# RS2002/PianoBart

Measured on AMD Instinct MI355X. Metric: Octuple tokens/sec/GPU (seq=1024, 12L/768d) pretrain step; %MFMA peak, higher is better.
Workload: dtype bf16

## Files before the change

pianobart_amd/csrc/pb_api_internal.h:

```cpp
#pragma once
#include <hip/hip_runtime.h>
#include "../../include/pianobart_hip.h"

int pb_gemm2_try(const pb_gemm_desc* d, void* stream);
int pb_finalize_rows(const float* partials, int nblk, int d, float* out, void* stream, int nacc = 1, float* out1 = nullptr);
float* pb_defer_alloc(size_t nfloats);
int pb_gemm_x3(const pb_gemm_desc* d, void* stream);
int pb_flash64_fwd(const pb_attn_desc& d, hipStream_t stream);
int pb_flash64_bwd(const pb_attn_desc& d, hipStream_t stream);
int pb_flash1_bwd(const pb_attn_desc& d, hipStream_t stream);
int pb_flash_x3_fwd(const pb_attn_desc& d, hipStream_t stream);
int pb_flash_x3_bwd(const pb_attn_desc& d, hipStream_t stream);
const void* pb_zero_page();
```

pianobart_amd/csrc/pb_gemm.hip:

```cpp
#include "pb_common.h"
#include "pb_api_internal.h"
#include <algorithm>

namespace {

constexpr int BM = 128, BN = 128, NTHREADS = 256;
constexpr int ROW_BYTES = 128;
constexpr int TILE_BYTES = BM * ROW_BYTES;

template <typename T> struct Elem;
template <> struct Elem<bf16_t> { static constexpr int EPV = 8, BK = 64; };
template <> struct Elem<float>  { static constexpr int EPV = 4, BK = 32; };

struct Vec16 { uint32_t w[4]; };

__device__ __forceinline__ int swz(int row) { return ((row >> 1) & 7) ^ ((row >> 4) & 7); }

template <typename T>
__device__ __forceinline__ Vec16 load_vec(const T* __restrict__ base, long off, int nvalid, bool aligned) {
    constexpr int EPV = Elem<T>::EPV;
    Vec16 v = {{0u, 0u, 0u, 0u}};
    if (nvalid <= 0) return v;
    if (aligned && nvalid == EPV) {
        const uint4 q = *reinterpret_cast<const uint4*>(base + off);
// ... 240 lines not shown
    else hipLaunchKernelGGL((gemm_kernel<T, false, false>), grid, block, lds, stream, a);
    PB_LAUNCH_CHECK();
    return 0;
}

}

static int colsum_of_c(const pb_gemm_desc* d, void* stream_) {
    const bool c32 = (d->flags & PB_GEMM_C_F32) || d->dtype == PB_F32;
    return pb_colsum(d->C, d->ldc, d->colsum_out, d->colsum_ws, d->M, d->N, c32 ? PB_F32 : PB_BF16, c32 ? 1 : 0, stream_);
}

extern "C" int pb_gemm(const pb_gemm_desc* d, void* stream_) {
    hipStream_t stream = (hipStream_t)stream_;
    PB_REQUIRE(d != nullptr, "pb_gemm: null descriptor");
    PB_REQUIRE(d->dtype == PB_F32 || d->dtype == PB_BF16 || d->dtype == PB_F32X3, "pb_gemm: bad dtype %d", d->dtype);
    PB_REQUIRE(d->M >= 0 && d->N >= 0 && d->K >= 0, "pb_gemm: negative size");
    if (d->M == 0 || d->N == 0) return 0;
    PB_REQUIRE(d->A && d->B && d->C, "pb_gemm: null operand");
    PB_REQUIRE(!(d->flags & PB_GEMM_GELU) || d->aux_out, "pb_gemm: GELU epilogue needs aux_out");
    PB_REQUIRE(!(d->flags & PB_GEMM_MUL_GELU_GRAD) || d->aux_in, "pb_gemm: gelu-grad epilogue needs aux_in");
    const int nbt = (d->nb1 > 0 ? d->nb1 : 1) * (d->nb2 > 0 ? d->nb2 : 1);
    PB_REQUIRE(!d->colsum_out || (d->colsum_ws && nbt == 1 && d->ldc == d->N && d->N % 4 == 0), "pb_gemm: colsum_out needs colsum_ws, one batch and a dense C with N a multiple of 4");
    if (d->dtype == PB_F32X3) return pb_gemm_x3(d, stream_);
    if (!(d->flags & PB_GEMM_FORCE_V1)) {
        const int r2 = pb_gemm2_try(d, stream_);
        if (r2 < 0) return r2;
        if (r2 == 0) return 0;
        if (r2 == 2) return colsum_of_c(d, stream_);
    }
    if (d->flags & PB_GEMM_ROWDOT) {
        pb_set_error("pb_gemm: PB_GEMM_ROWDOT is only served by the bf16 NT 256x256 kernel (not with PB_GEMM_FORCE_V1, f32, K %% 64 != 0 or operands off 16 bytes)");
        return -2;
    }
    const int esz = d->dtype == PB_BF16 ? 2 : 4, epv = 16 / esz;
    GemmArgs a;
    a.A = d->A; a.B = d->B; a.C = d->C; a.bias = d->bias; a.aux_in = d->aux_in; a.aux_out = d->aux_out;
    a.M = d->M; a.N = d->N; a.K = d->K; a.lda = d->lda; a.ldb = d->ldb; a.ldc = d->ldc; a.ldaux = d->ldaux;
    const int nb1 = d->nb1 > 0 ? d->nb1 : 1;
    a.nb2 = d->nb2 > 0 ? d->nb2 : 1;
    a.sA1 = d->sA1; a.sA2 = d->sA2; a.sB1 = d->sB1; a.sB2 = d->sB2; a.sC1 = d->sC1; a.sC2 = d->sC2;
    a.alpha = d->alpha; a.flags = d->flags;
    auto aligned = [&](const void* p, long ld, long s1, long s2) {
        return ((uintptr_t)p % 16 == 0) && (ld % epv == 0) && (s1 % epv == 0) && (s2 % epv == 0);
    };
    a.a_aligned = aligned(d->A, d->lda, d->sA1, d->sA2);
    a.b_aligned = aligned(d->B, d->ldb, d->sB1, d->sB2);
    a.tiles_m = (d->M + BM - 1) / BM; a.tiles_n = (d->N + BN - 1) / BN;
    PB_REQUIRE((long)nb1 * a.nb2 <= 65535, "pb_gemm: too many batches");
    const int rc = d->dtype == PB_BF16 ? launch_gemm<bf16_t>(a, d->a_kcontig, d->b_kcontig, nb1 * a.nb2, stream)
                                       : launch_gemm<float>(a, d->a_kcontig, d->b_kcontig, nb1 * a.nb2, stream);
    if (rc) return rc;
    return d->colsum_out ? colsum_of_c(d, stream_) : 0;
}

extern "C" int64_t pb_gemm_colsum_ws_floats(int32_t M, int32_t N) {
    const int64_t fused = 2LL * ((M + 255) / 256) * N;
    return std::max<int64_t>(fused, pb_colsum_partials_floats(N));
}
```

pianobart_amd/embedding.py:

```python
from collections import OrderedDict

import numpy as np
import torch

from . import ops, pieces
from ._lib import PBError

STAGES = ('encode', 'pool', 'moments', 'distances', 'knn', 'counts')
D2_BLOCK_BYTES = 64 << 20


def _run(timer, stage, fn, *args, **kw):
    return fn(*args, **kw) if timer is None else timer.run(stage, fn, *args, **kw)


class EmbeddingMixin:
    def embed(self, enc16, emask, timer=None):
        if enc16.device.type != 'cuda':
            raise PBError('pianobart_amd needs HIP device tensors (got %s); there is no CPU path' % enc16.device)
        B, S = int(enc16.shape[0]), int(enc16.shape[1])
        if emask is not None and tuple(emask.shape) != (B, S):
            raise PBError('embed: encoder_attention_mask of shape %s for ids of (%d, %d, 8)' % (tuple(emask.shape), B, S))
        self.bind(enc16.device)
        self._await_updates(2)
        with torch.no_grad():
            enc16 = self.note_ids(enc16.contiguous(), owned=False)
            em = emask.to(torch.float32).contiguous() if emask is not None else None
            _, enc_h = _run(timer, 'encode', self.forward_hidden, enc16, None, em, None, False, 0)
            emb, count = _run(timer, 'pool', ops.pool_rows, enc_h.view(B, S, self.d), em)
        self.check_ids(collective=False)
        return emb, count


def _backbone(model):
    pb = getattr(model, 'pianobart', model)
    if not hasattr(pb, 'embed') or not hasattr(pb, 'layout'):
        raise PBError('embedding: the model must be a PianoBart or a model that holds one as .pianobart (got %s)' % type(model).__name__)
    return pb


def arrange(ids, layout, pad_word, start=None):
    a = pieces.host_ids(ids, layout)
    live = pieces.live_rows(a, layout, start)[1]
    order = np.argsort(~live, axis=1, kind='stable')
    moved = np.take_along_axis(a, order[:, :, None], 1)
    n_live = live.sum(1)
    moved[np.arange(a.shape[1])[None, :] >= n_live[:, None]] = np.asarray(pad_word, dtype=np.int64)
    keep = n_live > 0
    return moved[keep], n_live[keep].astype(np.int64), int((~keep).sum())


def _embed_rows(pb, rows, batch_size, timer=None):
    if isinstance(batch_size, bool) or not isinstance(batch_size, (int, np.integer)) or batch_size < 1:
        raise PBError('embedding: batch_size = %r must be an integer >= 1' % (batch_size,))
    S = rows.shape[1]
    if S > pb.bartConfig.max_position_embeddings:
        raise PBError('embedding: pieces of %d rows exceed max_position_embeddings %d' % (S, pb.bartConfig.max_position_embeddings))
# ... 142 lines not shown
```

pianobart_amd/engine.py:

```python
import os

import numpy as np
import torch

from . import ops, rowpack

from ._lib import LIB, PB_BF16, PB_F32, PB_F32X3, PBError
from .generation import LN_EPS, GenerationMixin, check_prefix, check_samples, sample_seed
from .embedding import EmbeddingMixin
from .scoring import ScoringMixin

_WGRAD_STREAM = int(os.environ.get('PB_WGRAD_STREAM', '7'))
_WG_DXD_256 = int(os.environ.get('PB_WG_DXD_256', '1'))
_WG_TARGET = 192 if _WGRAD_STREAM & 1 else 256
_ROWDOT = int(os.environ.get('PB_ROWDOT', '1'))
_X3_ONEHOT = int(os.environ.get('PB_X3_ONEHOT', '1'))
_DP_RESERVE_CUS = int(os.environ.get('PB_DP_RESERVE_CUS', '0'))
_SIDE_PRIORITY = int(os.environ.get('PB_SIDE_PRIORITY', '0'))
_X3_FLASH = int(os.environ.get('PB_X3_FLASH', '1'))

_RING = 2
_EVENT_MODE = 1
_FWD_GEMM_FLAGS = int(os.environ.get('PB_FWD_GEMM_FLAGS', '32768'))
_PACK_ROWS = int(os.environ.get('PB_PACK_ROWS', '1'))
# ... 210 lines not shown
                    R, C = s.shape
                    rows.append([s.off, R, C, tiles])
                    tiles += -(-R // 64) * -(-C // 64)
                    self.wT[name] = self.PbfT[s.off:s.off + s.numel].view(C, R)
            if rows:
                self._wT_table = torch.tensor(rows, dtype=torch.int32, device=device)
                self._wT_tiles = tiles
        self.Gcur = self.G32
        self.opt_m = self.opt_v = None
        self._versions = None
        self._ws_cache = {}
        self.ptab = torch.zeros(self.lay.tab_total, self.d, dtype=torch.float32, device=device)
        self.dptab = torch.zeros(self.lay.tab_total, self.d, dtype=torch.float32, device=device)
        npart = max(int(LIB.query('pb_ln_partials_floats', self.d)), int(LIB.query('pb_colsum_partials_floats', max(3 * self.d, self.fe, self.fd, self.lay.vocab))),
                    int(LIB.query('pb_ce_partials_floats')), int(LIB.query('pb_norm_partials_floats')))
        self.partials = torch.empty(npart, dtype=torch.float32, device=device)
        self.scal = torch.zeros(64, dtype=torch.float32, device=device)
        w = [len(self.pb.e2w[k]) for k in self.pb.e2w]
        self.loss_w = torch.tensor(w, dtype=torch.float32, device=device)
        self.sos16 = torch.tensor(self.pb.sos_word_np, dtype=torch.int16, device=device)

    def _alias_cross_kv(self, dct):
        if self.ND:
            d2 = 2 * self.d
            for l in range(self.ND):
                dct['dec.%d.wkv_c' % l] = dct['dec.wkv_all'][l * d2:(l + 1) * d2]
                dct['dec.%d.bkv_c' % l] = dct['dec.bkv_all'][l * d2:(l + 1) * d2]

    def refresh_shadow(self, force=False):
        if self.code != PB_BF16:
            return
        ver = sum(p._version for p in self.params)
        if force or ver != self._versions:
            self._await_updates(2)
            ops.cast_f32_to_bf16(self.P32, self.Pbf)
            self._versions = ver
            self._shadow_gen += 1

    def _refresh_wT(self, on_side=False):
        if self._wT_table is None:
            return
        gen = self._shadow_gen
        if on_side and self._side and _WGRAD_STREAM:
            self._event().wait_on(self._side)
            with torch.cuda.stream(self._side):
                ops.transpose_batch_bf16(self.Pbf, self.PbfT, self._wT_table, self._wT_tiles)
                self._wT_done = self._event()
        else:
            ops.transpose_batch_bf16(self.Pbf, self.PbfT, self._wT_table, self._wT_tiles)
            self._wT_done = None
        self._wT_gen = gen

    def _ensure_wT(self):
        if self._wT_table is None:
            return
        if self._wT_gen != self._shadow_gen:
            self._refresh_wT()
        if self._wT_done is not None:
            self._wT_done.wait_on(torch.cuda.current_stream())
            self._wT_done = None

    def _ws(self, B, S):
        key = (B, S)
        ws = self._ws_cache.get(key)
        if ws is not None:
            return ws
        dev, X, d, H = self.device, self.xdt, self.d, self.H
# ... 135 lines not shown
    def forward_hidden(self, enc16, dec16, emask, dmask, train, seed, reuse_encoder=False, dec_embeds=None, pack=None):
        B, S = (pack.B, pack.S) if pack is not None else enc16.shape[:2]
        if S > self.Smax:
            raise PBError('sequence length %d exceeds max_position_embeddings %d' % (S, self.Smax))
        self._fwd_token += 1
        d = self.d
        Te, Td = (pack.Te, pack.Td) if pack is not None else (B * S, B * S)
        ws = self._ws_rows(self._ws(B, S), Te, Td)
        self._cur_ws = ws
        r_enc, r_dec, r_cross = (pack.enc, pack.dec, pack.cross) if pack is not None else (None, None, None)
        ids_e, ids_d = (pack.src_e, pack.src_d) if pack is not None else (None, None)
        p = self.p_drop if train else 0.0
        self._await_updates(0)
        if not self._tables_ready:
            self.refresh_shadow()
            self.build_ptab()
        self._tables_ready = False
        self._kmax = {}
        if self.use_flash and (self.x3 or self.hd in (64, 96, 128)) and pack is None:
            for msk in (emask, dmask):
                if msk is not None and id(msk) not in self._kmax:
                    km = torch.empty(msk.shape[0], dtype=torch.int32, device=msk.device)
                    ops.key_extent(msk, km)
                    self._kmax[id(msk)] = km
        self._kmax_keep = (emask, dmask)
        wf = self.wf
        x = ws['x_enc']
        if not reuse_encoder:
            ops.embed_ln_fwd(enc16, self.ptab, wf['lin.b'], wf['enc.pos'], wf['enc.lne.w'], wf['enc.lne.b'], x, ws['me'], ws['re'], S,
                             LN_EPS, seed, self._site('enc_emb'), p, padded=True, layout=self.lay, row_ids=ids_e)
        T = Te
        for l in range(self.NE if not reuse_encoder else 0):
            L, pf = ws['enc'][l], 'enc.%d.' % l
            if l == 2:
                self._await_updates(1)
            self._linear(x, pf + 'wqkv', pf + 'bqkv', L['qkv'], T, 3 * d, d)
            self._attn_fwd((L['qkv'], 0, 3 * d), (L['qkv'], d, 3 * d), (L['qkv'], 2 * d, 3 * d), (L['ctx'], 0, d), emask, False, B, S, S, L['attn'],
                           rows=r_enc)
            self._linear(L['ctx'], pf + 'wo', pf + 'bo', L['a1'], T, d, d)
            ops.add_ln_fwd(x, L['a1'], wf[pf + 'ln1.w'], wf[pf + 'ln1.b'], L['y1'], L['m1'], L['r1'], LN_EPS, seed, self._site('enc', l, 0), p, row_ids=ids_e)
            self._linear(L['y1'], pf + 'w1', pf + 'b1', L['g'], T, self.fe, d, gelu_aux_out=L['u'])
            self._linear(L['g'], pf + 'w2', pf + 'b2', L['a2'], T, d, self.fe)
            ops.add_ln_fwd(L['y1'], L['a2'], wf[pf + 'ln2.w'], wf[pf + 'ln2.b'], L['y2'], L['m2'], L['r2'], LN_EPS, seed, self._site('enc', l, 1), p, row_ids=ids_e)
            x = L['y2']
        enc_out = x if not reuse_encoder else (ws['enc'][-1]['y2'] if self.NE else x)
        if dec16 is None and dec_embeds is None:
            return None, enc_out
        self._await_updates(2)
        y = ws['x_dec']
        T = Td
        if dec_embeds is None:
            ops.embed_ln_fwd(dec16, self.ptab, wf['lin.b'], wf['dec.pos'], wf['dec.lne.w'], wf['dec.lne.b'], y, ws['md'], ws['rd'], S,
                             LN_EPS, seed, self._site('dec_emb'), p, padded=True, layout=self.lay, row_ids=ids_d)
        else:
            ws['alt_pos'] = wf['dec.pos'][2:2 + S].to(self.xdt).unsqueeze(0).expand(B, S, d).reshape(T, d).contiguous()
            ws['alt_e'] = dec_embeds
            pre = y if p == 0.0 else ws.setdefault('x_dec_pre', torch.empty_like(y))
            ops.add_ln_fwd(ws['alt_pos'], dec_embeds, wf['dec.lne.w'], wf['dec.lne.b'], pre, ws['md'], ws['rd'], LN_EPS, 0, 0, 0.0)
            if p > 0.0:
                ops.dropout(pre, y, seed, self._site('dec_emb'), p)
        kvld = self.ND * 2 * d
        kv_cut = min(_KV_CUT, self.ND)

        def kv_project(l0, l1):
            ops.gemm(enc_out, self.w['dec.wkv_all'], ws['kvc_all'], M=Te, N=(l1 - l0) * 2 * d, K=d, dtype=self.gcode, bias=self.wf['dec.bkv_all'][l0 * 2 * d:],
                     ldc=kvld, b_off=l0 * 2 * d * d, c_off=l0 * 2 * d, dbg=_FWD_GEMM_FLAGS)
        kv_ready = None
        if (_WGRAD_STREAM & 2) and self._side_stream() is not None and self.ND:
            self._event().wait_on(self._side)
            with torch.cuda.stream(self._side):
                kv_project(0, kv_cut)
                kv_ready = [self._event()] * kv_cut
                if self.ND > kv_cut:
                    kv_project(kv_cut, self.ND)
                    kv_ready += [self._event()] * (self.ND - kv_cut)
        elif self.ND:
            kv_project(0, self.ND)
        kv_of = lambda l: ((ws['kvc_all'], l * 2 * d, kvld), (ws['kvc_all'], l * 2 * d + d, kvld))
        sub = pack.sub if pack is not None else None
        sub_layer = None
        for l in range(self.ND):
# ... 321 lines not shown
            gA = self._ffn_ln_bwd(L, pf, self.fe, cur, L['y1'], seed, self._site('enc', l, 1), p, Te, row_ids=ids_e)
            dqkv_e = self._ring('dqkv')[:Te]
            g2 = gy if cur is not gy else galt
            bq = g[pf + 'bqkv']
            fused = self._attn_block_bwd(L, pf, (pf + 'wo', pf + 'bo'), gA, x_in, (L['qkv'], 0, 3 * d), (L['qkv'], d, 3 * d), (L['qkv'], 2 * d, 3 * d),
                                         (dqkv_e, 0, 3 * d), (dqkv_e, d, 3 * d), (dqkv_e, 2 * d, 3 * d), L['ctx'], L['a1'], L['attn'],
                                         L['m1'], L['r1'], wf[pf + 'ln1.w'], g[pf + 'ln1.b'], g[pf + 'ln1.w'], g2, seed, self._site('enc', l, 0), p, B, S, S, emask, False,
                                         dbias=(bq[:d], bq[d:2 * d], bq[2 * d:]), T=Te, rows=r_enc, row_ids=ids_e)
            if not fused:
                ops.colsum(dqkv_e, bq, self.partials, Te, 3 * d)
            self._wgrad(dqkv_e, x_in, pf + 'wqkv', 3 * d, d, Te)
            self._dgrad(dqkv_e, pf + 'wqkv', g2, Te, d, 3 * d, True)
            cur = g2
            self._ready(pf + 'wqkv', pf + 'w2')
        side_tail = (_WGRAD_STREAM & 1) and self._side_stream() is not None and self.grad_hook is None
        if side_tail:
            self._event().wait_on(self._side)
            with torch.cuda.stream(self._side):
                ops.defer_flush()
                self._side_last = self._event()
        ops.embed_ln_bwd(cur, sv['enc16'], self.ptab, wf['lin.b'], wf['enc.pos'], wf['enc.lne.w'], ws['me'], ws['re'], self.dptab,
                         g['enc.pos'], g['lin.b'], g['enc.lne.w'], g['enc.lne.b'], self.partials, S, seed, self._site('enc_emb'), p,
                         dz_out=ws['dz'][:Te] if onehot_route else None, padded=True, layout=self.lay, row_ids=pack.src_e if pack is not None else None)
        if onehot_route:
            if pack is not None:
                ops.pos_grad_packed(ws['dz'][:Te], pack.inv_e, g['enc.pos'][2:2 + S], B, S)
            else:
                ops.batch_sum(ws['dz'][:T], g['enc.pos'][2:2 + S], B, S * d)
            ops.onehot_build(sv['enc16'], ws['onehot'][:Te], padded=True, layout=self.lay)
            if dec_tab_done is not None:
                dec_tab_done.wait_on(torch.cuda.current_stream())
            self._onehot_gemm(ws['onehot'][:Te], ws['dz'][:Te], Te, dec_tab_done is not None, side=False)
        E, W, R = self.wf['emb'], self.wf['lin.w'], self.lay.tab_rows
        lin_w = lambda: ops.gemm(self.dptab, E, g['lin.w'], M=d, N=256, K=R, dtype=PB_F32, a_kc=False, b_kc=False, lda=d, ldb=256, ldc=2048, alpha=16.0,
                                 c_f32=True, nb1=8, sA=(R * d, 0), sB=(R * 256, 0), sC=(256, 0))
        if side_tail:
            self._event().wait_on(self._side)
            with torch.cuda.stream(self._side):
                lin_w()
                self._side_last = self._event()
        ops.gemm(self.dptab, W, g['emb'], M=R, N=256, K=d, dtype=PB_F32, b_kc=False, lda=d, ldb=2048, ldc=256, alpha=16.0, c_f32=True,
                 nb1=8, sA=(R * d, 0), sB=(256, 0), sC=(R * 256, 0))
        if not side_tail:
            lin_w()
        self._ready('emb', 'lin.w')
        if not side_tail:
            ops.defer_flush()
        self._join_side()
        if self.grad_hook is not None and self.Gcur is self.G32 and not (self._micro is not None and self._micro[0] < self._micro[1] - 1):
            self._add_accumulated(self.n_matrix, self.n_total)
            self.grad_hook(self.n_matrix, self.n_total)

    def _onehot_gemm(self, onehot, dz, K, accum, side):
        d = self.d
        which = 1 if side else 0
        need = 16 * self.lay.tab_total * d
        if self._slabs_oh[which] is None:
            self._slabs_oh[which] = torch.empty(need, dtype=torch.float32, device=self.device)
        one = lambda b, acc: ops.gemm(onehot, b, self.dptab, M=self.lay.tab_total, N=d, K=K, dtype=PB_BF16, a_kc=False, b_kc=False, lda=self.lay.tab_total, ldb=d,
                                      dbg=self._bwd_dbg(), ldc=d, c_f32=True, accum=acc, splitk=16, slabs=self._slabs_oh[which], tile256=True)
        if self.x3:
            planes = self._cur_ws.get('_base', self._cur_ws)['dz_planes']
            r0 = (dz.data_ptr() - self._cur_ws.get('_base', self._cur_ws)['dz'].data_ptr()) // (4 * d)
            hi, lo = planes[0, r0:r0 + K], planes[1, r0:r0 + K]

            def launch():
                ops.split_bf16(dz[:K], hi, lo)
                one(hi, accum)
                one(lo, True)
        else:
            launch = lambda: one(dz, accum)
        if side and (_WGRAD_STREAM & 1) and self._side_stream() is not None:
            self._event().wait_on(self._side)
            with torch.cuda.stream(self._side):
                launch()
                done = self._event()
            self._side_last = done
# ... 267 lines not shown
            self.opt_v = torch.zeros_like(self.P32)
        self.step_count += 1
        sq, clip = self.scal[40:41], self.scal[41:42]
        ops.grad_sqnorm(self.G32, self.partials, sq)
        ops.clip_coef(sq, max_norm, gscale, clip)
        if self.pipeline_updates and self.code == PB_BF16 and _WGRAD_STREAM and self._side_stream() is not None:
            self._event().wait_on(self._side)
            with torch.cuda.stream(self._side):
                evs = []
                for ranges in self._update_groups():
                    for lo, hi in ranges:
                        ops.adamw_step(self.P32[lo:hi], self.G32[lo:hi], self.opt_m[lo:hi], self.opt_v[lo:hi], self.Pbf[lo:hi], clip, lr, betas[0], betas[1],
                                       eps, weight_decay, self.step_count)
                    evs.append(self._event())
                self._versions = sum(p._version for p in self.params)
                self._shadow_gen += 1
                if self._wT_table is not None:
                    ops.transpose_batch_bf16(self.Pbf, self.PbfT, self._wT_table, self._wT_tiles)
                    self._wT_done = self._event()
                    self._wT_gen = self._shadow_gen
            self._upd, self._upd_waited = evs, 0
            return
        ops.adamw_step(self.P32, self.G32, self.opt_m, self.opt_v, self.Pbf, clip, lr, betas[0], betas[1], eps, weight_decay, self.step_count)
        if self.code == PB_BF16:
            self._versions = sum(p._version for p in self.params)
            self._shadow_gen += 1
            self._refresh_wT(on_side=True)

    def _update_groups(self):
        if self._upd_groups is None:
            first = lambda names: next((self.slots[n].off for n in names if n in self.slots), self.n_matrix)
            a2 = first(['dec.0.wqkv', 'head.w'])
            a1 = min(first(['enc.2.wqkv']), a2)
            self._upd_groups = [[(0, a1), (self.n_matrix, self.n_total)], [(a1, a2)], [(a2, self.n_matrix)]]
            self._upd_groups = [[(lo, hi) for lo, hi in g if hi > lo] for g in self._upd_groups]
        return self._upd_groups

    def _await_updates(self, group=2):
        if self._upd is None:
            return
        cur = torch.cuda.current_stream()
        while self._upd_waited <= group:
            self._upd[self._upd_waited].wait_on(cur)
            self._upd_waited += 1
        if self._upd_waited >= len(self._upd):
            self._upd = None

    def finish_updates(self):
        self._await_updates(2)



class _LMFn(torch.autograd.Function):

    @staticmethod
    def forward(ctx, eng, enc_ids, dec_ids, emask, dmask, training, need_grad, *params):
        enc16, dec16, em, dm = eng._prep_inputs(enc_ids, dec_ids, emask, dmask)
        B, S = enc16.shape[:2]
        seed = eng._next_seed() if training else 0
        dec_h, _ = eng.forward_hidden(enc16, dec16, em, dm, training, seed)
        logits = eng.heads_forward(dec_h)
        eng._fwd_token += 1
        ctx.eng, ctx.token = eng, eng._fwd_token
        out = logits.view(B, S, eng.lay.vocab)
        return out.clone()

    @staticmethod
    def backward(ctx, dlogits):
        eng = ctx.eng
        if ctx.token != eng._fwd_token:
            raise PBError('backward for a stale forward: the engine keeps the activations of the most recent forward only')
        ws = eng._cur_ws
        T = ws['T']
        p0 = eng.params[0]
        alias = p0.grad is not None and p0.grad.data_ptr() == eng.grad_views[0].data_ptr()
        eng._select_grads(alias)
        dl = dlogits.reshape(T, eng.lay.vocab).contiguous()
        if eng.xdt == torch.float32:
            dlx = dl.float()
        else:
            dlx = ws['dlogits']
            ops.cast_f32_to_bf16(dl.float().contiguous(), dlx)
# ... 50 lines not shown
```

pianobart_amd/generation.py:

```python
import contextlib
import os
import time
from types import SimpleNamespace

import numpy as np
import torch

from . import ops
from ._lib import LIB, PB_BF16, PBError

_DECODE_SPEC = int(os.environ.get('PB_DECODE_SPEC', '1'))
_DECODE_GRAPH = int(os.environ.get('PB_DECODE_GRAPH', '1'))

LN_EPS = 1e-5


def check_prefix(prefix, prefix_len, B, S, pad):
    if prefix is None:
        if prefix_len is not None and any(int(v) for v in (prefix_len.tolist() if hasattr(prefix_len, 'tolist') else prefix_len)):
            raise PBError('prefix_len given without a prefix')
        return [0] * B, None
    p = torch.as_tensor(prefix)
    if p.dim() != 3 or int(p.shape[0]) != B or int(p.shape[2]) != 8:
        raise PBError('prefix of shape %s: expected (%d, P, 8) for %d prompt(s)' % (tuple(p.shape), B, B))
# ... 519 lines not shown
    return forced


def sample_seed(seed, j, i, N):
    return int(seed) + int(j) * int(N) + int(i)


def sampler_form_for(sizes, p):
    ranked = sum(int(n) for n, q in zip(sizes, p) if float(q) < 1.0)
    return 'wide' if max(int(n) for n in sizes) > 272 or ranked > 512 else 'narrow'


class GenerationMixin:
    last_sampler_form = None

    def _note_sampler_form(self, dec):
        self.last_sampler_form = 'wide' if int(LIB.query('pb_batch_decoder_sampler_form', dec)) else 'narrow'
        return dict(sampler_form='wide') if self.last_sampler_form == 'wide' else {}

    def generate(self, enc_ids, emask, sample_row, use_cache=True, max_new=None, sampler=None, prefix=None, forced=None, stop=None, order=None, allow=None):
        S = int(enc_ids.shape[1])
        with_ended = stop is not None
        ks, rows = check_prefix(prefix, None, 1, S, self.pb.pad_word_np)
        forced = check_forced(forced, 1, S, list(self.lay.sizes) if forced is not None else None, ks)
        stop = check_stop([stop] if isinstance(stop, (int, np.integer)) and not isinstance(stop, bool) else stop, 1, int(self.pb.pad_word_np[0]))
        sb = stop[0] if stop is not None else None
        order = check_order([order] if isinstance(order, (int, np.integer)) and not isinstance(order, bool) else order, 1, order_max=int(self.pb.pad_word_np[0]) - 1)
        ob = order[0] if order is not None else None
        allow = check_allow(allow, 1, self.lay if allow is not None else None)
        ab = unpack_allow(allow, self.lay.vocab)[0] if allow is not None else None
        fr = forced[0] if forced is not None else None
        k = ks[0]
        pre = rows[0, :k] if k else None
        self._await_updates(2)
        if not use_cache:
            return self._generate_nocache(enc_ids, emask, sample_row, k, pre, fr, sb, ob, ab)
        if self.hd not in (32, 64, 96, 128):
            return self._generate_pyloop(enc_ids, emask, sample_row, k, pre, fr, sb, ob, ab)
        with torch.no_grad(), self._decoder_run(enc_ids, emask, ks, rows, round2=True) as run:
            self.last_decode = None
            res_cpu, pad_cpu = run.res_cpu, run.pad_cpu
            if run.dec is not None:
                if sampler is not None and _DECODE_SPEC:
                    fault = int(getattr(self, 'decode_fault_period', 0) or 0)
                    info = self._decode_device_sampled(run.dec, 1, S, lambda b, row, **kw: sample_row(row, **kw), [np.random.get_state()], sampler,
                                                       res_cpu, pad_cpu, max_new, (0, fault), inline_verify=True, starts=[k], forced=forced, stop=stop,
                                                       order=order, allow=allow)
                    info.update(tokens=info['tokens'][0], rewinds=info['rewinds'][0], ended=info['ended'][0])
                else:
                    info = self._decode_host_sampled(run.dec, S, sample_row, res_cpu, pad_cpu, max_new, k, fr, sb, ob, ab)
                self.last_decode = dict(info, s_enc=run.s_enc[0], prefix=k, prefill_ms=float(run.prefill_ms()))
                if not with_ended:
                    del self.last_decode['ended']
            else:
                import ctypes
                pref, stream = ctypes.byref(run.bp.plan), ops._stream()
                tok16 = run.bufs['tok16']
                if k:
                    tok16.copy_(pre[k - 1].to(torch.int16))
                tok_pin = torch.empty(8, dtype=torch.int16).pin_memory()
                logit_pin = torch.empty(self.lay.vocab, dtype=torch.float32).pin_memory()
                sv = stop_vector(pad_cpu, sb)
                prev = pre[k - 1] if k else torch.from_numpy(self.pb.sos_word_np)
                for i in range(k, S):
                    LIB.call('pb_decode_step', pref, i, stream)
                    logit_pin.copy_(run.bufs['logits'][0])
                    tok = allowed_token(fr[i] if fr is not None else None, lambda **kw: sample_row(logit_pin, **kw), ab, ob, prev, pad_cpu)
# ... 146 lines not shown
        n = 0
        t_loop = time.perf_counter()
        for i in range(k, S if max_new is None else min(S, k + max_new)):
            LIB.call('pb_batch_decoder_step', dec, tok_p, log_p)
            n += 1
            tok = allowed_token(fr[i] if fr is not None else None, lambda **kw: sample_row(logit_cpu, **kw), allow, order, tok_np, pad_cpu)
            if (tok >= sv).any():
                ended = end_reason(tok, pad_cpu)
                break
            res_cpu[0, i] = tok
            tok_np[:] = tok.numpy()
        return dict(launches_per_token=int(LIB.query('pb_batch_decoder_launches', dec)), graph=bool(LIB.query('pb_batch_decoder_graph', dec)),
                    tokens=n, loop_ms=(time.perf_counter() - t_loop) * 1e3, ended=ended)

    BATCH_MAX = 16

    def generate_batch(self, enc_ids, emask, sample_row, rngs, max_new=None, sampler=None, prefix=None, prefix_len=None, samples=None, forced=None,
                       refill=False, stop=None, order=None, allow=None):
        def done(out, with_ended=stop is not None):
            if not with_ended and self.last_decode is not None:
                self.last_decode.pop('ended', None)
            return out
        P = int(enc_ids.shape[0])
        slots = check_refill(refill, samples, self.BATCH_MAX)
        owner = check_samples(samples, P, len(rngs)) if samples is not None else list(range(P))
        ks, rows = check_prefix(prefix, prefix_len, P, int(enc_ids.shape[1]), self.pb.pad_word_np)
        forced = check_forced(forced, P, int(enc_ids.shape[1]), list(self.lay.sizes) if forced is not None else None, ks)
        pad0 = int(self.pb.pad_word_np[0])
        stop = check_stop(stop, P, pad0, owner if samples is not None else None)
        order = check_order(order, P, owner if samples is not None else None, order_max=pad0 - 1)
        allow = check_allow(allow, P, self.lay if allow is not None else None, owner if samples is not None else None)
        if len(rngs) != len(owner):
            raise PBError('generate_batch: %d generators for %d prompts' % (len(rngs), P))
        self._await_updates(2)
        R = len(owner)
        if R == 0:
            return torch.from_numpy(self.pb.pad_word_np).to(enc_ids.device).repeat(0, enc_ids.shape[1], 1)
        if not self._batch_decoder_covers(sampler):
            if samples is None:
                return done(self._generate_batch_loop(enc_ids, emask, sample_row, rngs, max_new, sampler, ks, rows, forced, stop, order, allow))
            return done(self._generate_batch_expanded(enc_ids, emask, sample_row, rngs, max_new, sampler, ks, rows, owner, forced, stop, order, allow))
        if slots and R > slots:
            out = self._generate_batch_refill(enc_ids, emask, sample_row, rngs, max_new, sampler, ks, rows, forced, slots, stop, order, allow)
            if out is not None:
                return done(out)
        outs, ended = [], []
        for c0 in range(0, R, self.BATCH_MAX):
            own = owner[c0:c0 + self.BATCH_MAX]
            st = stop[c0:c0 + len(own)] if stop is not None else None
            st = st if st is not None and any(v != pad0 for v in st) else None
            od = order[c0:c0 + len(own)] if order is not None else None
            od = od if od is not None and any(v != -1 for v in od) else None
            al = _slice_allow(allow, c0, c0 + len(own))
            p0, p1 = own[0], own[-1] + 1
            outs.append(self._generate_batch_chunk(enc_ids[p0:p1], emask[p0:p1] if emask is not None else None, sample_row,
                                                   rngs[c0:c0 + len(own)], max_new, sampler, ks[p0:p1], rows[p0:p1] if rows is not None else None,
                                                   groups=[p - p0 for p in own] if samples is not None else None,
                                                   forced=forced[p0:p1] if forced is not None and (forced[p0:p1] != -1).any() else None, stop=st, order=od,
                                                   allow=al))
            ended += (self.last_decode or {}).get('ended') or [None] * len(own)
        if len(outs) > 1 and self.last_decode is not None:
            self.last_decode['ended'] = ended
        return done(torch.cat(outs, 0))

    def _generate_batch_expanded(self, enc_ids, emask, sample_row, rngs, max_new, sampler, ks, rows, owner, forced=None, stop=None, order=None,
                                 allow=None):
        idx = torch.as_tensor(owner, dtype=torch.long)
# ... 471 lines not shown
```

pianobart_amd/scoring.py:

```python
from types import SimpleNamespace

import numpy as np
import torch

from . import ops
from ._lib import PBError


def _int_list(v):
    return [int(x) for x in (v.tolist() if hasattr(v, 'tolist') else list(v))]


def default_length(target_ids, bar_pad):
    t = torch.as_tensor(target_ids)
    live = (t[:, :, 0] != int(bar_pad)).to(torch.int64)
    return _int_list(live.cumprod(1).sum(1))


def check_score_args(input_ids_encoder, target_ids, start=None, length=None, max_positions=None, bar_pad=None):
    e, t = torch.as_tensor(input_ids_encoder), torch.as_tensor(target_ids)
    for name, x in (('input_ids_encoder', e), ('target_ids', t)):
        if x.dim() != 3 or int(x.shape[2]) != 8:
            raise PBError('score: %s of shape %s: expected (B, S, 8)' % (name, tuple(x.shape)))
        if x.dtype.is_floating_point or x.dtype.is_complex or x.dtype == torch.bool:
# ... 19 lines not shown
        for b, x in enumerate(vals):
            if isinstance(x, bool) or not isinstance(x, (int, np.integer)):
                raise PBError('score: %s[%d] = %r is not an integer' % (name, b, x))
        out.append([int(x) for x in vals])
    start, length = out
    for b in range(B):
        if not 0 <= start[b] <= length[b] <= S:
            raise PBError('score: row %d: start = %d, length = %d outside 0 <= start <= length <= %d' % (b, start[b], length[b], S))
    return start, length


def pick_best(scores):
    s = np.asarray(scores, dtype=np.float64)
    if s.ndim != 3 or s.shape[2] != 9:
        raise PBError('pick_best: scores of shape %s: expected (N, n, 9)' % (s.shape,))
    total, count = s[:, :, :8].sum(-1), s[:, :, 8]
    with np.errstate(divide='ignore', invalid='ignore'):
        key = np.where(count > 0, total / np.where(count > 0, count, 1.0), -np.inf)
    return np.argmax(key, axis=1).astype(np.int64)


class ScoringMixin:
    def score(self, enc16, tgt16, emask, start, length):
        if self.mlm is None:
            raise PBError('engine has no LM heads')
        if enc16.device.type != 'cuda':
            raise PBError('pianobart_amd needs HIP device tensors (got %s); there is no CPU path' % enc16.device)
        B, S = int(tgt16.shape[0]), int(tgt16.shape[1])
        start, length = _int_list(start), _int_list(length)
        if len(start) != B or len(length) != B or any(not 0 <= s <= n <= S for s, n in zip(start, length)):
            raise PBError('score: start / length need %d entries with 0 <= start <= length <= %d' % (B, S))
        dev = enc16.device
        self.bind(dev)
        self._await_updates(2)
        with torch.no_grad():
            enc16 = self.note_ids(enc16.contiguous(), owned=False)
            tgt16 = self.note_ids(tgt16.contiguous(), owned=False)
            em = emask.to(torch.float32).contiguous() if emask is not None else None
            pos = torch.arange(S, device=dev).unsqueeze(0)
            st = torch.tensor(start, device=dev).unsqueeze(1)
            ln = torch.tensor(length, device=dev).unsqueeze(1)
            mask = ((pos >= st) & (pos < ln)).to(torch.float32).contiguous()
            dmask = (pos < ln.clamp(min=1)).to(torch.float32).contiguous()
            dec16 = torch.empty_like(tgt16)
            ops.shift_right(tgt16, self.sos16, dec16, B, S)
            dec_h, _ = self.forward_hidden(enc16, dec16, em, dmask, False, 0)
            logits = self.heads_forward(dec_h)
            logp = torch.empty(B, S, 8, dtype=torch.float32, device=dev)
            entropy = torch.empty(B, S, 8, dtype=torch.float32, device=dev)
            rank = torch.empty(B, S, 8, dtype=torch.int16, device=dev)
            sums = torch.empty(B, 4, 8, dtype=torch.float32, device=dev)
            ops.token_scores(logits, tgt16.view(B * S, 8), mask.view(B * S), logp, entropy, rank, layout=self.lay)
            ops.seq_scores(logp, entropy, rank, mask, sums)
        self.check_ids(collective=False)
        return SimpleNamespace(logp=logp, entropy=entropy, rank=rank, sum_logp=sums[:, 0], sum_entropy=sums[:, 1], hits=sums[:, 2],
                               count=sums[:, 3, 0])
```

Measured before the change: 636,400.

## Add small f32 GEMM kernel, split update groups finer, serialize embedding weight grads

```diff
diff --git a/pianobart_amd/csrc/pb_api_internal.h b/pianobart_amd/csrc/pb_api_internal.h
--- a/pianobart_amd/csrc/pb_api_internal.h
+++ b/pianobart_amd/csrc/pb_api_internal.h
@@ -3,6 +3,8 @@
 #include "../../include/pianobart_hip.h"
 
 int pb_gemm2_try(const pb_gemm_desc* d, void* stream);
+int pb_gemm_small_try(const pb_gemm_desc* d, void* stream);
+extern "C" int pb_gemm_small_route(const pb_gemm_desc* d);
 int pb_finalize_rows(const float* partials, int nblk, int d, float* out, void* stream, int nacc = 1, float* out1 = nullptr);
 float* pb_defer_alloc(size_t nfloats);
 int pb_gemm_x3(const pb_gemm_desc* d, void* stream);
diff --git a/pianobart_amd/csrc/pb_gemm.hip b/pianobart_amd/csrc/pb_gemm.hip
--- a/pianobart_amd/csrc/pb_gemm.hip
+++ b/pianobart_amd/csrc/pb_gemm.hip
@@ -296,6 +296,10 @@
     if (d->flags & PB_GEMM_ROWDOT) {
         pb_set_error("pb_gemm: PB_GEMM_ROWDOT is only served by the bf16 NT 256x256 kernel (not with PB_GEMM_FORCE_V1, f32, K %% 64 != 0 or operands off 16 bytes)");
         return -2;
+    }
+    {
+        const int rs = pb_gemm_small_try(d, stream_);
+        if (rs <= 0) return rs;
     }
     const int esz = d->dtype == PB_BF16 ? 2 : 4, epv = 16 / esz;
     GemmArgs a;
diff --git a/pianobart_amd/csrc/pb_gemm_route.h b/pianobart_amd/csrc/pb_gemm_route.h
--- /dev/null
+++ b/pianobart_amd/csrc/pb_gemm_route.h
@@ -0,0 +1,21 @@
+#pragma once
+#include <stdint.h>
+#include "../../include/pianobart_hip.h"
+
+#define PB_GEMM_SMALL_MAX_TILES 160
+#define PB_GEMM_SMALL_MAX_K 1024
+
+static inline int pb_gemm_vec16_ok(const void* p, int64_t ld, int64_t s1, int64_t s2) {
+    return ((uintptr_t)p % 16 == 0) && (ld % 4 == 0) && (s1 % 4 == 0) && (s2 % 4 == 0);
+}
+
+static inline int pb_gemm_small_rule(const pb_gemm_desc* d) {
+    if (d->dtype != PB_F32) return 0;
+    if (d->flags & (PB_GEMM_FORCE_V1 | PB_GEMM_GELU | PB_GEMM_MUL_GELU_GRAD | PB_GEMM_NO_EPILOGUE | PB_GEMM_ROWDOT)) return 0;
+    if (d->bias || d->colsum_out) return 0;
+    if (d->splitk > 1 && d->slabs) return 0;
+    if (d->M <= 0 || d->N <= 0 || d->K < 4 || d->K % 4 != 0 || d->K > PB_GEMM_SMALL_MAX_K) return 0;
+    const int64_t tm = ((int64_t)d->M + 127) / 128, tn = ((int64_t)d->N + 127) / 128, nb1 = d->nb1 > 0 ? d->nb1 : 1, nb2 = d->nb2 > 0 ? d->nb2 : 1;
+    if (tm > PB_GEMM_SMALL_MAX_TILES || tn > PB_GEMM_SMALL_MAX_TILES || nb1 > PB_GEMM_SMALL_MAX_TILES || nb2 > PB_GEMM_SMALL_MAX_TILES) return 0;
+    return tm * tn * nb1 * nb2 <= PB_GEMM_SMALL_MAX_TILES;
+}
diff --git a/pianobart_amd/csrc/pb_gemm_small.hip b/pianobart_amd/csrc/pb_gemm_small.hip
--- /dev/null
+++ b/pianobart_amd/csrc/pb_gemm_small.hip
@@ -0,0 +1,160 @@
+#include "pb_common.h"
+#include "pb_api_internal.h"
+#include "pb_gemm_route.h"
+
+namespace {
+
+constexpr int TM = 64, TN = 64, TK = 32, NTHREADS = 256;
+constexpr int PITCH = 64 + 16;
+constexpr int OPER = TK * PITCH;
+
+struct SmallArgs {
+    const float* A; const float* B; float* C;
+    int M, N, K;
+    long lda, ldb, ldc;
+    int nb2; long sA1, sA2, sB1, sB2, sC1, sC2;
+    float alpha;
+    int accum, a_aligned, b_aligned, tiles_m;
+};
+
+__device__ __forceinline__ f32x4 load_vec4(const float* __restrict__ base, long off, int nvalid, bool aligned) {
+    f32x4 v = {0.f, 0.f, 0.f, 0.f};
+    if (nvalid <= 0) return v;
+    if (aligned && nvalid >= 4) return *reinterpret_cast<const f32x4*>(base + off);
+#pragma unroll
+    for (int j = 0; j < 4; ++j)
+        if (j < nvalid) v[j] = base[off + j];
+    return v;
+}
+
+template <bool KC>
+__device__ __forceinline__ void gload(f32x4 (&v)[4], const float* __restrict__ base, long ld, int r0, int k0, int R, int K, bool aligned, int b) {
+    if constexpr (KC) {
+        const int gk = k0 + 4 * (b & 7);
+#pragma unroll
+        for (int i = 0; i < 4; ++i) {
+            const int gr = r0 + 4 * (b >> 3) + i;
+            v[i] = load_vec4(base, (long)gr * ld + gk, gr < R ? K - gk : 0, aligned);
+        }
+    } else {
+        const int gr = r0 + 4 * (b & 15);
+#pragma unroll
+        for (int i = 0; i < 4; ++i) {
+            const int gk = k0 + 4 * (b >> 4) + i;
+            v[i] = load_vec4(base, (long)gk * ld + gr, gk < K ? R - gr : 0, aligned);
+        }
+    }
+}
+template <bool KC>
+__device__ __forceinline__ void lstore(const f32x4 (&v)[4], float* lds, int b) {
+    if constexpr (KC) {
+        float* p = lds + 4 * (b & 7) * PITCH + 4 * (b >> 3);
+#pragma unroll
+        for (int j = 0; j < 4; ++j) *reinterpret_cast<f32x4*>(p + j * PITCH) = f32x4{v[0][j], v[1][j], v[2][j], v[3][j]};
+    } else {
+        float* p = lds + 4 * (b >> 4) * PITCH + 4 * (b & 15);
+#pragma unroll
+        for (int i = 0; i < 4; ++i) *reinterpret_cast<f32x4*>(p + i * PITCH) = v[i];
+    }
+}
+
+template <bool A_KC, bool B_KC>
+__global__ __launch_bounds__(NTHREADS) void gemm_small_kernel(const SmallArgs p) {
+    __shared__ __attribute__((aligned(16))) float smem[2 * 2 * OPER];
+    const int t = threadIdx.x, lane = t & 63, wave = t >> 6;
+    const int wm = wave >> 1, wn = wave & 1, lr = lane & 15, lg = lane >> 4;
+    const int tm = blockIdx.x % p.tiles_m, tn = blockIdx.x / p.tiles_m;
+    const int m0 = tm * TM, n0 = tn * TN;
+    const int z = blockIdx.y, z1 = z / p.nb2, z2 = z % p.nb2;
+    const float* A = p.A + z1 * p.sA1 + z2 * p.sA2;
+    const float* B = p.B + z1 * p.sB1 + z2 * p.sB2;
+    float* C = p.C + z1 * p.sC1 + z2 * p.sC2;
+    const bool for_b = t >= 128;
+    const int b = t & 127;
+
+    f32x4 acc[2][2];
+#pragma unroll
+    for (int i = 0; i < 2; ++i)
+#pragma unroll
+        for (int j = 0; j < 2; ++j) acc[i][j] = f32x4{0.f, 0.f, 0.f, 0.f};
+
+    f32x4 v[4];
+    auto load = [&](int k0) {
+        if (for_b) gload<B_KC>(v, B, p.ldb, n0, k0, p.N, p.K, p.b_aligned, b);
+        else gload<A_KC>(v, A, p.lda, m0, k0, p.M, p.K, p.a_aligned, b);
+    };
+    auto store = [&](float* stage) {
+        if (for_b) lstore<B_KC>(v, stage + OPER, b);
+        else lstore<A_KC>(v, stage, b);
+    };
+
+    const int nk = (p.K + TK - 1) / TK;
+    load(0);
+    store(smem);
+    __syncthreads();
+    for (int kt = 0; kt < nk; ++kt) {
+        float* cur = smem + (kt & 1) * 2 * OPER;
+        const bool more = kt + 1 < nk;
+        if (more) load((kt + 1) * TK);
+        const int nkb = min(TK, p.K - kt * TK) >> 2;
+        const float* la = cur + lg * PITCH + wm * 32 + lr;
+        const float* lb = cur + OPER + lg * PITCH + wn * 32 + lr;
+#pragma unroll
+        for (int kb = 0; kb < TK / 4; ++kb) {
+            if (kb < nkb) {
+                const float a0 = la[4 * kb * PITCH], a1 = la[4 * kb * PITCH + 16];
+                const float b0 = lb[4 * kb * PITCH], b1 = lb[4 * kb * PITCH + 16];
+                acc[0][0] = __builtin_amdgcn_mfma_f32_16x16x4f32(a0, b0, acc[0][0], 0, 0, 0);
+                acc[0][1] = __builtin_amdgcn_mfma_f32_16x16x4f32(a0, b1, acc[0][1], 0, 0, 0);
+                acc[1][0] = __builtin_amdgcn_mfma_f32_16x16x4f32(a1, b0, acc[1][0], 0, 0, 0);
+                acc[1][1] = __builtin_amdgcn_mfma_f32_16x16x4f32(a1, b1, acc[1][1], 0, 0, 0);
+            }
+        }
+        if (more) store(smem + ((kt + 1) & 1) * 2 * OPER);
+        __syncthreads();
+    }
+
+#pragma unroll
+    for (int j = 0; j < 2; ++j) {
+        const int col = n0 + wn * 32 + j * 16 + lr;
+        if (col >= p.N) continue;
+#pragma unroll
+        for (int i = 0; i < 2; ++i) {
+#pragma unroll
+            for (int r = 0; r < 4; ++r) {
+                const int row = m0 + wm * 32 + i * 16 + lg * 4 + r;
+                if (row >= p.M) continue;
+                float* c = C + (long)row * p.ldc + col;
+                float val = p.alpha * acc[i][j][r] + 0.f;
+                if (p.accum) val += *c;
+                *c = val;
+            }
+        }
+    }
+}
+
+}
+
+extern "C" int pb_gemm_small_route(const pb_gemm_desc* d) { return pb_gemm_small_rule(d); }
+
+int pb_gemm_small_try(const pb_gemm_desc* d, void* stream_) {
+    if (!pb_gemm_small_rule(d)) return 1;
+    const int nb1 = d->nb1 > 0 ? d->nb1 : 1, nb2 = d->nb2 > 0 ? d->nb2 : 1;
+    SmallArgs a;
+    a.A = (const float*)d->A; a.B = (const float*)d->B; a.C = (float*)d->C;
+    a.M = d->M; a.N = d->N; a.K = d->K; a.lda = d->lda; a.ldb = d->ldb; a.ldc = d->ldc;
+    a.nb2 = nb2; a.sA1 = d->sA1; a.sA2 = d->sA2; a.sB1 = d->sB1; a.sB2 = d->sB2; a.sC1 = d->sC1; a.sC2 = d->sC2;
+    a.alpha = d->alpha; a.accum = (d->flags & PB_GEMM_ACCUM) ? 1 : 0;
+    a.a_aligned = pb_gemm_vec16_ok(d->A, d->lda, d->sA1, d->sA2);
+    a.b_aligned = pb_gemm_vec16_ok(d->B, d->ldb, d->sB1, d->sB2);
+    a.tiles_m = (d->M + TM - 1) / TM;
+    const int tiles_n = (d->N + TN - 1) / TN;
+    dim3 grid(a.tiles_m * tiles_n, nb1 * nb2), block(NTHREADS);
+    hipStream_t stream = (hipStream_t)stream_;
+    if (d->a_kcontig && d->b_kcontig) hipLaunchKernelGGL((gemm_small_kernel<true, true>), grid, block, 0, stream, a);
+    else if (d->a_kcontig && !d->b_kcontig) hipLaunchKernelGGL((gemm_small_kernel<true, false>), grid, block, 0, stream, a);
+    else if (!d->a_kcontig && d->b_kcontig) hipLaunchKernelGGL((gemm_small_kernel<false, true>), grid, block, 0, stream, a);
+    else hipLaunchKernelGGL((gemm_small_kernel<false, false>), grid, block, 0, stream, a);
+    PB_LAUNCH_CHECK();
+    return 0;
+}
diff --git a/pianobart_amd/embedding.py b/pianobart_amd/embedding.py
--- a/pianobart_amd/embedding.py
+++ b/pianobart_amd/embedding.py
@@ -22,7 +22,7 @@
         if emask is not None and tuple(emask.shape) != (B, S):
             raise PBError('embed: encoder_attention_mask of shape %s for ids of (%d, %d, 8)' % (tuple(emask.shape), B, S))
         self.bind(enc16.device)
-        self._await_updates(2)
+        self._await_updates()
         with torch.no_grad():
             enc16 = self.note_ids(enc16.contiguous(), owned=False)
             em = emask.to(torch.float32).contiguous() if emask is not None else None
diff --git a/pianobart_amd/engine.py b/pianobart_amd/engine.py
--- a/pianobart_amd/engine.py
+++ b/pianobart_amd/engine.py
@@ -266,7 +266,7 @@
             return
         ver = sum(p._version for p in self.params)
         if force or ver != self._versions:
-            self._await_updates(2)
+            self._await_updates()
             ops.cast_f32_to_bf16(self.P32, self.Pbf)
             self._versions = ver
             self._shadow_gen += 1
@@ -468,8 +468,8 @@
         T = Te
         for l in range(self.NE if not reuse_encoder else 0):
             L, pf = ws['enc'][l], 'enc.%d.' % l
-            if l == 2:
-                self._await_updates(1)
+            if l == 0 or l == 2:
+                self._await_updates(1 if l == 0 else 2)
             self._linear(x, pf + 'wqkv', pf + 'bqkv', L['qkv'], T, 3 * d, d)
             self._attn_fwd((L['qkv'], 0, 3 * d), (L['qkv'], d, 3 * d), (L['qkv'], 2 * d, 3 * d), (L['ctx'], 0, d), emask, False, B, S, S, L['attn'],
                            rows=r_enc)
@@ -482,7 +482,7 @@
         enc_out = x if not reuse_encoder else (ws['enc'][-1]['y2'] if self.NE else x)
         if dec16 is None and dec_embeds is None:
             return None, enc_out
-        self._await_updates(2)
+        self._await_updates()
         y = ws['x_dec']
         T = Td
         if dec_embeds is None:
@@ -870,17 +870,10 @@
                 dec_tab_done.wait_on(torch.cuda.current_stream())
             self._onehot_gemm(ws['onehot'][:Te], ws['dz'][:Te], Te, dec_tab_done is not None, side=False)
         E, W, R = self.wf['emb'], self.wf['lin.w'], self.lay.tab_rows
-        lin_w = lambda: ops.gemm(self.dptab, E, g['lin.w'], M=d, N=256, K=R, dtype=PB_F32, a_kc=False, b_kc=False, lda=d, ldb=256, ldc=2048, alpha=16.0,
-                                 c_f32=True, nb1=8, sA=(R * d, 0), sB=(R * 256, 0), sC=(256, 0))
-        if side_tail:
-            self._event().wait_on(self._side)
-            with torch.cuda.stream(self._side):
-                lin_w()
-                self._side_last = self._event()
         ops.gemm(self.dptab, W, g['emb'], M=R, N=256, K=d, dtype=PB_F32, b_kc=False, lda=d, ldb=2048, ldc=256, alpha=16.0, c_f32=True,
                  nb1=8, sA=(R * d, 0), sB=(256, 0), sC=(R * 256, 0))
-        if not side_tail:
-            lin_w()
+        ops.gemm(self.dptab, E, g['lin.w'], M=d, N=256, K=R, dtype=PB_F32, a_kc=False, b_kc=False, lda=d, ldb=256, ldc=2048, alpha=16.0,
+                 c_f32=True, nb1=8, sA=(R * d, 0), sB=(R * 256, 0), sC=(256, 0))
         self._ready('emb', 'lin.w')
         if not side_tail:
             ops.defer_flush()
@@ -1214,13 +1207,16 @@
             first = lambda names: next((self.slots[n].off for n in names if n in self.slots), self.n_matrix)
             a2 = first(['dec.0.wqkv', 'head.w'])
             a1 = min(first(['enc.2.wqkv']), a2)
-            self._upd_groups = [[(0, a1), (self.n_matrix, self.n_total)], [(a1, a2)], [(a2, self.n_matrix)]]
+            a0 = min(first(['enc.0.wqkv']), a1)
+            self._upd_groups = [[(0, a0), (self.n_matrix, self.n_total)], [(a0, a1)], [(a1, a2)], [(a2, self.n_matrix)]]
             self._upd_groups = [[(lo, hi) for lo, hi in g if hi > lo] for g in self._upd_groups]
         return self._upd_groups
 
-    def _await_updates(self, group=2):
+    def _await_updates(self, group=None):
         if self._upd is None:
             return
+        if group is None:
+            group = len(self._upd) - 1
         cur = torch.cuda.current_stream()
         while self._upd_waited <= group:
             self._upd[self._upd_waited].wait_on(cur)
@@ -1229,7 +1225,7 @@
             self._upd = None
 
     def finish_updates(self):
-        self._await_updates(2)
+        self._await_updates()
 
 
 
diff --git a/pianobart_amd/generation.py b/pianobart_amd/generation.py
--- a/pianobart_amd/generation.py
+++ b/pianobart_amd/generation.py
@@ -575,7 +575,7 @@
         fr = forced[0] if forced is not None else None
         k = ks[0]
         pre = rows[0, :k] if k else None
-        self._await_updates(2)
+        self._await_updates()
         if not use_cache:
             return self._generate_nocache(enc_ids, emask, sample_row, k, pre, fr, sb, ob, ab)
         if self.hd not in (32, 64, 96, 128):
@@ -788,7 +788,7 @@
         allow = check_allow(allow, P, self.lay if allow is not None else None, owner if samples is not None else None)
         if len(rngs) != len(owner):
             raise PBError('generate_batch: %d generators for %d prompts' % (len(rngs), P))
-        self._await_updates(2)
+        self._await_updates()
         R = len(owner)
         if R == 0:
             return torch.from_numpy(self.pb.pad_word_np).to(enc_ids.device).repeat(0, enc_ids.shape[1], 1)
diff --git a/pianobart_amd/scoring.py b/pianobart_amd/scoring.py
--- a/pianobart_amd/scoring.py
+++ b/pianobart_amd/scoring.py
@@ -75,7 +75,7 @@
             raise PBError('score: start / length need %d entries with 0 <= start <= length <= %d' % (B, S))
         dev = enc16.device
         self.bind(dev)
-        self._await_updates(2)
+        self._await_updates()
         with torch.no_grad():
             enc16 = self.note_ids(enc16.contiguous(), owned=False)
             tgt16 = self.note_ids(tgt16.contiguous(), owned=False)
```

Result: no change. 638,700, median of 6 (+0.4%).
